# theadamsabra/last_torch

Hardware: AMD Instinct MI355X
Metric: lattice cells/s (B·T·U·|ctx|) at T=1000,U=100; 1/2/4/8-GPU scaling (higher is better)
Workload: dtype f32; 1 GPU; Log-semiring forward-backward (loss + dW), B=64/GPU, T=1000, U=100, V=32, FullNGram n=1 (C=33), fp32 (BASELINE configs[1]; configs[2] at 8 GPUs); batch_per_gpu=64, global_batch=64, frames=1000, labels=100, vocab=32, context_size=1, context_states=33, parallelism=utterance-sharded x1 (LPT), one RCCL all-reduce per step

## Files before the change

last_torch_amd/csrc/lt_chunk.hip:

```cpp
#include "lt_kernels.h"

#include <unistd.h>

#include <atomic>
#include <chrono>

namespace {

typedef float v16f __attribute__((ext_vector_type(16)));

constexpr float kEmin = 0x1p-88f;
constexpr int kRec = 1248;
constexpr int kRowT = 36;
constexpr int kChunkLds = 40 * 1024;
constexpr int kMargWaves = 4;
constexpr int kGrp = 7;
constexpr float kCert = 64.f;
#ifndef LT_AB_WAVES
#define LT_AB_WAVES 3
#endif
constexpr int kAbWaves = LT_AB_WAVES;
#ifndef LT_CK_APF
#define LT_CK_APF 1
#endif
constexpr int kApf = LT_CK_APF;
static_assert(kApf == 1 || kApf == 2, "phase A prefetch depth");
constexpr unsigned kSpinMax = 1u << 20;
#ifndef LT_CK_SPLIT
#define LT_CK_SPLIT 0
#endif
#ifndef LT_CK_WPRIO
#define LT_CK_WPRIO 3
#endif
#ifndef LT_CK_PRIO
#define LT_CK_PRIO 3
#endif
#ifndef LT_CK_ROT
#define LT_CK_ROT 1
#endif
#ifndef LT_CK_PF
#define LT_CK_PF 0
#endif
#ifndef LT_CK_NOACQ
#define LT_CK_NOACQ 1
#endif
constexpr bool kNoAcq = LT_CK_NOACQ != 0;
#ifndef LT_CK_ALDS
#define LT_CK_ALDS 1
#endif
constexpr bool kALds = LT_CK_ALDS != 0;
constexpr int kASlot = 5 * 1024;
constexpr int kALdsBytes = 4 * 2 * kASlot;
#ifndef LT_CK_BANDMIX
#define LT_CK_BANDMIX 0
#endif
constexpr bool kBandMix = LT_CK_BANDMIX != 0;
#ifndef LT_CK_EPIPE
#define LT_CK_EPIPE 0
#endif
constexpr bool kEpipe = LT_CK_EPIPE != 0;
#ifndef LT_WALK_SLOTS
#define LT_WALK_SLOTS 3
#endif
constexpr int kWalkSlots = LT_WALK_SLOTS;
constexpr int kRecNi = (4 * kRec + 1023) / 1024;
constexpr int kWalkSlot = kRecNi * 1024;
constexpr int kWalkLds = 2 * kWalkSlots * kWalkSlot;
constexpr int kRecEj = 1152, kRecRt = 1184, kRecRho = 1216, kRecPi = 1217, kRecCs = 1218,
              kRecFlag = 1219, kRecN = 1220;

struct CkArgs {
  const unsigned char* W;
  const int* nfr;
  const int* labels;
  const int* nlab;
  const float* grad;
  float* rec;
  float* nb;
  int* uflag;
  float* abd;
  float* bbd;
  float* nabd;
  float* nbbd;
  float* cf;
  unsigned long long* ready;
  unsigned long long* prog;
  unsigned long long ep_tag, pg_tag;
  float* mid;
  float* loss;
  float* log_z;
  float* num;
  float* lz_out;
  float* num_out;
  void* dW;
  int B, T, U, V, C, R, FR, NP, NPG, PPL, CP;
  int L, K;
  int NGc;
  int nc, wpos;
  int nbs;
  int half;
  int cont;
  int local;
  int strict;
  int dbg;
  int pf;
  long long* stamps;
  long long FB;
  int a_slots, a_ni, a_slot_bytes, a_wave_bytes, a_off_rt, a_off_tab;
  int b_ni, b_slots, b_off_ra, b_off_rb, b_off_ga, b_off_gb, b_gslots, b_gslot, b_off_buf;
  int c_ni, c_off_ad, c_off_bd, c_off_an, c_off_bn, c_off_nw, c_off_fs, c_off_tab, c_off_cf,
      c_off_buf, c_off_fl, c_off_e, c_bytes;
};

LT_DEVINL float half_sum(float v) {
  auto p = __builtin_amdgcn_permlane32_swap(__float_as_int(v), __float_as_int(v), false, false);
  return __int_as_float(p[0]) + __int_as_float(p[1]);
}
LT_DEVINL float half_other(float v) {
  auto p = __builtin_amdgcn_permlane32_swap(__float_as_int(v), __float_as_int(v), false, false);
  return (threadIdx.x & 32) ? __int_as_float(p[0]) : __int_as_float(p[1]);
}
LT_DEVINL float from_prev(float v, float fill) {
  return __int_as_float(
      __builtin_amdgcn_update_dpp(__float_as_int(fill), __float_as_int(v), 0x138, 0xF, 0xF, false));
}
LT_DEVINL float rot_prev(float v) {
  return __int_as_float(__builtin_amdgcn_update_dpp(0, __float_as_int(v), 0x13C, 0xF, 0xF, false));
}
LT_DEVINL float rot_next(float v) {
  return __int_as_float(__builtin_amdgcn_update_dpp(0, __float_as_int(v), 0x134, 0xF, 0xF, false));
}

LT_DEVINL float safe_max(float m) { return __builtin_isfinite(m) ? m : 0.f; }
#ifdef LT_DIAG
#define CK_STAMP(k)                                                                  \
  do {                                                                               \
    if (a.stamps && !LT_ABL(a, 64 | 256) && threadIdx.x == 0)                         \
      a.stamps[(long long)blockIdx.x * 8 + (k)] = (long long)__builtin_amdgcn_s_memtime(); \
  } while (0)
#define CK_WSTAMP(k)                                                                 \
  do {                                                                               \
    if (a.stamps && LT_ABL(a, 64) && (threadIdx.x & 63) == 0)                         \
      a.stamps[(long long)b * 8 + (k)] = (long long)__builtin_amdgcn_s_memtime();     \
  } while (0)
#define CK_ASTAMP(k)                                                                 \
  do {                                                                               \
    if (a.stamps && LT_ABL(a, 256) && (threadIdx.x & 63) == 0)                        \
      a.stamps[(long long)a.B * a.K * 8 + (long long)id * 4 + (k)] =                  \
          (long long)__builtin_amdgcn_s_memtime();                                   \
  } while (0)
#else
#define CK_ASTAMP(k) \
  do {               \
  } while (0)
#define CK_WSTAMP(k) \
  do {               \
  } while (0)
#define CK_STAMP(k) \
  do {              \
  } while (0)
#endif
LT_DEVINL float max3_raw(float x, float y, float z) {
  float r;
  asm("v_max3_f32 %0, %1, %2, %3" : "=v"(r) : "v"(x), "v"(y), "v"(z));
  return r;
}
LT_DEVINL float first_lane(float v) {
  return __int_as_float(__builtin_amdgcn_readfirstlane(__float_as_int(v)));
}

LT_DEVINL int kstep(int s, int h) { return (s & 3) + 8 * (s >> 2) + 4 * h; }

template <bool BF16>
LT_DEVINL float ldsw(const unsigned char* fr, int e) {
  if constexpr (BF16) return __uint_as_float(((unsigned)((const unsigned short*)fr)[e]) << 16);
  else return ((const float*)fr)[e];
}

LT_DEVINL void dma_issue(const unsigned char* base, long long off, long long bytes,
                         unsigned lds_addr, int ni, int lane, int wave0 = 0, int nwaves = 1,
                         bool sc1 = false) {
  const long long a0 = off & ~15LL;
  const int n16 = (int)((off + bytes - a0 + 15) >> 4);
  for (int i = wave0; i < ni; i += nwaves) {
    int g = lane + 64 * i;
    g = g < n16 ? g : n16 - 1;
    if (sc1) glds16_sc1(base + a0 + 16LL * g, lds_addr + 1024u * i);
    else glds16(base + a0 + 16LL * g, lds_addr + 1024u * i);
  }
}

LT_DEVINL void pf_lines(const unsigned char* base, long long off, long long bytes,
                        unsigned lds_addr, int lane) {
  const long long a0 = off & ~127LL;
  const int nl = (int)((off + bytes - a0 + 127) >> 7);
  lds_addr = __builtin_amdgcn_readfirstlane(lds_addr);
  for (int i = 0; 64 * i < nl; ++i) {
    const int g = min(lane + 64 * i, nl - 1);
    const void* src = base + a0 + 128LL * g;
    unsigned keep;
    asm volatile(
        "s_mov_b32 %0, m0\n\t"
        "s_mov_b32 m0, %2\n\t"
        "s_nop 0\n\t"
        "global_load_lds_dword %1, off\n\t"
        "s_mov_b32 m0, %0"
        : "=&s"(keep)
        : "v"(src), "s"(lds_addr)
        : "memory");
  }
}

LT_DEVINL void dma_range(const unsigned char* base, long long off, long long bytes,
// ... 873 lines not shown
      if (lane == 0) a.mid[2LL * b] = O;
    } else {
      if (wt) prog_publish(a, b, 0, k1 - Kh, lane);
      const float x = lane < C ? al : -kInf;
      const float M = safe_max(wmax_u(x));
      const float s = wsum_u(lane < C ? __builtin_amdgcn_exp2f(x - M) : 0.f);
      if (lane == 0)
        *wl.lz = (float)(((double)O + (double)(M + __builtin_amdgcn_logf(s))) * 0.6931471805599453);
    }
  } else if (wave == 1 && !a.local && !LT_ABL(a, 1)) {
    float* bc = wl.bc + 64;
    const int h = lane >> 5;
    float* dst = a.bbd + (long long)b * (a.K + 1) * CP;
    const int k0 = ph == kWalkFirst ? Kh : 0, k1 = ph == kWalkRest ? Kh : Kl;
    float be;
    if (ph == kWalkRest) {
      const float x = dst[(long long)Kh * CP + min(lane, C - 1)];
      be = lane < C ? x : -kInf;
    } else {
      be = lane < C ? 0.f : -kInf;
      if (lane < C) dst[(long long)Kl * CP + lane] = be;
    }
    int pub = 0;
    if (k1 > k0) {
      rd.ensure_bwd(k1 - kWalkSlots, lane);
      for (int n = 0; n < kWalkSlots; ++n) issue_rec(k1 - 1 - n, n);
    }
    for (int n = 0; n < k1 - k0; ++n) {
      const int k = k1 - 1 - n;
      wait_rec(n);
      RecBeta R;
      load_rec_beta(slot(n), lane, R);
      const float xc = (lane >= 1 && lane < C) ? be : -kInf;
      const float Mc = safe_max(wmax_u(xc));
      if (lane >= 1 && lane <= 32) bc[lane - 1] = lane < C ? __builtin_amdgcn_exp2f(xc - Mc) : 0.f;
      __builtin_amdgcn_s_waitcnt(0xc07f);
      __builtin_amdgcn_wave_barrier();
      float p0 = 0.f, p1 = 0.f;
#pragma unroll
      for (int g = 0; g < 4; ++g) {
        const float4 b4 = *(const float4*)(bc + 8 * g + 4 * h);
        p0 = __builtin_fmaf(R.x[4 * g + 0], b4.x, p0);
        p1 = __builtin_fmaf(R.x[4 * g + 1], b4.y, p1);
        p0 = __builtin_fmaf(R.x[4 * g + 2], b4.z, p0);
        p1 = __builtin_fmaf(R.x[4 * g + 3], b4.w, p1);
      }
      const float rp = lane < 32 ? R.rt * bc[lane & 31] : 0.f;
      const float ej = R.ej, rho = R.rho, pi = R.pi;
      __builtin_amdgcn_s_waitcnt(0xc07f);
      rd.ensure_bwd(k - kWalkSlots, lane);
      issue_rec(k - kWalkSlots, n + kWalkSlots);
      const float fl = floorf(Mc);
      const float tot = half_sum(p0 + p1);
      const float nj = (Mc - fl) + ej + __builtin_amdgcn_logf(tot);
      const float rsum = wsum_u(rp);
      const float rterm = (Mc - fl) + rho + __builtin_amdgcn_logf(rsum);
      const float nb0 = lse2_b2(first_lane(be) + pi - fl, rterm);
      const float sh = from_prev(nj, -kInf);
      be = lane == 0 ? nb0 : (lane < C ? sh : -kInf);
      if (lane < C) bd_store(dst + (long long)k * CP + lane, be, wt);
      if (wt && Kh - k - pub >= kProgStep && k > k0) {
        prog_publish(a, b, 1, Kh - k, lane);
        pub = Kh - k;
      }
      __builtin_amdgcn_wave_barrier();
    }
    if (wt) prog_publish(a, b, 1, Kh - k0, lane);
  } else if (wave == 2 && !LT_ABL(a, 2) && !LT_ABL(a, 128)) {
    num_walk<PPL, true, D>(a, b, lane, nf, Kl, nl, wl.nva, wl.num, rd, ph);
  } else if (wave == 3 && !LT_ABL(a, 2)) {
    num_walk<PPL, false, D>(a, b, lane, nf, Kl, nl, wl.nvb, nullptr, rd, ph);
  }
  if (lane == 0 && (rd.bad || !rd.ok)) *wl.bad = 1;
  CK_WSTAMP(2 * wave + 1);
  __syncthreads();
  if (ph == kWalkFirst) {
    if (threadIdx.x == 0) a.uflag[b] = *wl.bad ? 1 : 0;
    return;
  }
  if (*wl.bad) {
    if (threadIdx.x == 0) a.uflag[b] = 1;
    return;
  }
  if (threadIdx.x == 0) {
    const float lz = a.local ? 0.f : *wl.lz;
    const float nm = *wl.num;
    if (ph == kWalkRest && ((!a.local && !__builtin_isfinite(lz)) || !__builtin_isfinite(nm)))
      a.uflag[b] = 1;
    else if (ph == kWalkFull)
      a.uflag[b] = 0;
    a.log_z[b] = lz;
    a.num[b] = nm;
    if (a.lz_out) a.lz_out[b] = lz;
    if (a.num_out) a.num_out[b] = nm;
    a.loss[b] = a.local ? -nm : lz - nm;
  }
}

template <int PPL>
constexpr int kWalkD = PPL == 1 ? 8 : (kAbWaves > 3 ? 4 : 5);
template <int PPL>
constexpr int kWalkDc = PPL == 1 ? 4 : 3;

template <bool BF16, int PPL, bool FULL>
__global__ __launch_bounds__(256, kAbWaves) void ck_ab_kernel(const CkArgs a) {
  const int nc = a.nc;
  const int wave = __builtin_amdgcn_readfirstlane(threadIdx.x >> 6);
  int x = blockIdx.x;
  if (x >= a.wpos && x < a.wpos + nc) {
    extern __shared__ __attribute__((aligned(16))) unsigned char ck_dyn[];
    if (LT_CK_WPRIO) __builtin_amdgcn_s_setprio(LT_CK_WPRIO);
    combine_role<PPL, kWalkD<PPL>>(a, x - a.wpos, wave, ck_dyn, a.half ? kWalkFirst : kWalkFull);
    return;
  }
  if (x >= a.wpos) x -= nc;
  const long long j = (long long)x * 4 + wave;
  const int m = (int)(j / (2 * a.B));
  const int r = (int)(j - (long long)m * 2 * a.B);
  const int b = r < a.B ? r : r - a.B;
  int nf = a.nfr[b];
  nf = nf < 0 ? 0 : (nf > a.T ? a.T : nf);
  const int Kl = (nf + a.L - 1) / a.L;
  const int k = r < a.B ? m : Kl - 1 - m;
  if (r < a.B ? m > Kl - 1 - m : Kl - 1 - m <= m) return;
  transfer_role<BF16, PPL, FULL>(a, b, k, wave);
}

template <int PPL>
__global__ __launch_bounds__(256) void ck_combine_kernel(const CkArgs a) {
  extern __shared__ __attribute__((aligned(16))) unsigned char ck_dyn[];
  combine_role<PPL, kWalkD<PPL>>(a, blockIdx.x, __builtin_amdgcn_readfirstlane(threadIdx.x >> 6),
                                 ck_dyn, a.half ? kWalkFirst : kWalkFull);
}

LT_DEVINL void gather_tables(const CkArgs& a, int b, int* lab, int* boff, int* loff, int tid,
                             int nthr) {
  for (int j = tid; j < a.U; j += nthr) lab[j] = a.labels[(long long)b * a.U + j];
  __syncthreads();
  for (int u = tid; u < a.NPG; u += nthr) {
    int bo, lo;
    string_offsets(a, lab, u, &bo, &lo);
    boff[u] = bo < 0 ? 0 : bo;
    loff[u] = lo;
  }
}

template <bool BF16>
LT_DEVINL void store_dw(void* dW, long long e, float v) {
  if constexpr (BF16) ((unsigned short*)dW)[e] = f2bf(v);
  else ((float*)dW)[e] = v;
}

constexpr int kFs = 8, kFsMa = 0, kFsA0 = 1, kFsMb = 2, kFsB0 = 3, kFsW00 = 4;
constexpr int kFlA = 1, kFlB = 2, kFlNA = 4, kFlNB = 8, kFlAll = 15;

template <bool BF16, int PPL, bool FULL>
__global__ __launch_bounds__(64 * kMargWaves, kMargWaves / 2) void ck_marg_kernel(const CkArgs a) {
  extern __shared__ __attribute__((aligned(16))) unsigned char lds[];
  const int tid = threadIdx.x, lane = tid & 63;
  const int wave = __builtin_amdgcn_readfirstlane(tid >> 6);
  if (a.cont && (int)blockIdx.x < a.B) {
    CK_STAMP(0);
    if (LT_CK_WPRIO) __builtin_amdgcn_s_setprio(LT_CK_WPRIO);
    combine_role<PPL, kWalkDc<PPL>>(a, blockIdx.x, wave, lds, kWalkRest);
    CK_STAMP(4);
    return;
  }
  const int c = a.cont ? (int)blockIdx.x - a.B : (int)blockIdx.x;
  const int j = c / a.B, b = c - j * a.B;
  if (a.uflag[b]) return;
  int nf = a.nfr[b];
  nf = nf < 0 ? 0 : (nf > a.T ? a.T : nf);
  const int Kl = (nf + a.L - 1) / a.L, Kh = Kl / 2;
  const int k = j < 2 * Kh ? ((j & 1) ? Kh - 1 - (j >> 1) : Kh + (j >> 1)) : j;
  const int t0 = k * a.L;
  const int tend = min(t0 + a.L, a.T);
  const int t1 = max(t0, min(t0 + a.L, nf));
  const int V = FULL ? 32 : a.V, C = V + 1, R = V + 1, FR = C * R, CP = FULL ? 36 : a.CP;
  const int NPG = a.NPG, NP = a.NP;
  const int FRP = (FR + 3) & ~3;
  float g = a.grad ? a.grad[b] : 1.f;
  if (!a.cont) {
    const float lz = a.log_z[b], nm = a.num[b];
    if ((!a.local && !__builtin_isfinite(lz)) || __builtin_isnan(nm)) {
      if (tid == 0) a.uflag[b] = 1;
      return;
    }
    if (!__builtin_isfinite(nm)) g = 0.f;
  }
  const long long e0 = ((long long)b * a.T + t0) * FR;
  if (t1 <= t0 || g == 0.f) {
    const long long n = (long long)(tend - t0) * FR;
    for (long long e = tid; e < n; e += blockDim.x) store_dw<BF16>(a.dW, e0 + e, 0.f);
    return;
  }
  const int nt = t1 - t0;
  CK_STAMP(0);
  const int role = LT_CK_ROT == 1 ? (wave + (int)(blockIdx.x >> 3)) & 3
                 : LT_CK_ROT == 2 ? (wave + (int)blockIdx.x) & 3 : wave;
  const bool split = LT_CK_SPLIT && !a.local && !LT_ABL(a, 4 | 8);
  const int hs = (nt + 1) / 2;
  const long long off = e0 * (BF16 ? 2 : 4);
  if (!split) {
    dma_issue(a.W, off, (long long)nt * a.FB, lds_base_addr(lds), a.c_ni, lane, wave, kMargWaves);
  } else if (role < 2) {
    const int n1 = (int)(((off & 15) + (long long)hs * a.FB + 1023) >> 10);
    dma_range(a.W, off, (long long)nt * a.FB, lds_base_addr(lds), role == 0 ? 0 : max(n1 - 1, 0),
              role == 0 ? n1 : a.c_ni, lane);
  }
  unsigned char* wch = lds + (off & 15);
  float* xa = (float*)(lds + a.c_off_ad);
  float* xb = (float*)(lds + a.c_off_bd);
  float* an = (float*)(lds + a.c_off_an);
  float* bn = (float*)(lds + a.c_off_bn);
  float2* nw = (float2*)(lds + a.c_off_nw);
  float* fs = (float*)(lds + a.c_off_fs);
  int* boff = (int*)(lds + a.c_off_tab);
  int* loff = boff + NPG;
  int* labs = loff + NPG;
  float* buf = (float*)(lds + a.c_off_buf) + 64 * wave;
  float* cfl = (float*)(lds + a.c_off_cf);
  int* fl = (int*)(lds + a.c_off_fl);
  int* ford = fl + a.L;
  int* njob = ford + a.L;
  int* cert_fail = njob + 1;
  auto init_flags = [&](int t) {
    if (t < nt) {
      fl[t] = 0;
      const int mid = (nt - 1) / 2;
      const int k = (t + 1) / 2;
      ford[t] = (t & 1) ? mid + k : mid - k;
    }
    if (t == 0) {
      *njob = 0;
      *cert_fail = 0;
    }
  };
  if (split && role >= 2) {
    const int t2 = (role - 2) * 64 + lane;
    if (t2 < nt) cfl[t2] = a.cf[(long long)b * a.T + t0 + t2];
    for (int j = lane; j < a.U; j += 64) labs[j] = a.labels[(long long)b * a.U + j];
    __builtin_amdgcn_s_waitcnt(0xc07f);
    for (int u = t2; u < NPG; u += 128) {
      int bo, lo;
      string_offsets(a, labs, u, &bo, &lo);
      boff[u] = bo < 0 ? 0 : bo;
      loff[u] = lo;
    }
    init_flags(t2);
  }
  if (!split && tid < nt) cfl[tid] = a.cf[(long long)b * a.T + t0 + tid];
  if (a.cont && (split ? (role == 2 && lane == 0) : tid == 0)) {
    const int need_a = k - Kh, need_b = Kh - (k + 1);
    const unsigned long long* pg = a.prog + 4LL * b;
    int ok = 1;
    for (unsigned spins = 0;; ++spins) {
      bool done = true;
      if (need_a > 0)
        done = (a.local || prog_count(poll_flag(pg + 0), a.pg_tag) >= need_a) &&
               prog_count(poll_flag(pg + 2), a.pg_tag) >= need_a;
      if (done && need_b > 0)
        done = (a.local || prog_count(poll_flag(pg + 1), a.pg_tag) >= need_b) &&
               prog_count(poll_flag(pg + 3), a.pg_tag) >= need_b;
      if (done) break;
      if (spins > kSpinMax) {
        ok = 0;
        break;
      }
      __builtin_amdgcn_s_sleep(2);
    }
    if (!kNoAcq) acquire_agent();
    CK_STAMP(6);
    fl[2 * a.L + 2] = ok;
  }
  if (!split) {
    gather_tables(a, b, labs, boff, loff, tid, blockDim.x);
    wait_vmcnt(0);
    __syncthreads();
  } else {
    __builtin_amdgcn_s_waitcnt(0xc07f);
    __builtin_amdgcn_s_barrier();
    __builtin_amdgcn_fence(__ATOMIC_ACQUIRE, "workgroup");
  }
  if (a.cont && !fl[2 * a.L + 2]) {
    if (tid == 0) a.uflag[b] = 1;
    return;
  }
  CK_STAMP(1);
  auto wrow = [&](int f) -> const unsigned char* { return wch + f * a.FB; };
  auto eptr = [&](int f) -> float* {
    return BF16 ? (float*)(lds + a.c_off_e) + f * FRP : (float*)(wch + f * a.FB);
  };
  auto ew = [](float w, float cl) -> float {
    return __builtin_amdgcn_exp2f(__builtin_fmaf(w, kLog2e, -cl));
  };
  if (!split) {
    float2 g2[4];
    const int nnw = nt * NPG;
#pragma unroll
    for (int i = 0; i < 4; ++i) {
      const int x = min(tid + 64 * kMargWaves * i, nnw - 1);
      const int f = x / NPG, u = x - f * NPG;
      const unsigned char* fr = wch + f * a.FB;
      const int lo = loff[u];
      const float wb = ldsw<BF16>(fr, boff[u]), wl = ldsw<BF16>(fr, max(lo, 0));
      g2[i] = make_float2(u < NP ? wb * kLog2e : -kInf, (u >= 1 && u < NP) ? wl * kLog2e : -kInf);
    }
    for (int x = tid + 4 * 64 * kMargWaves; x < nnw; x += 64 * kMargWaves) {
      const int f = x / NPG, u = x - f * NPG;
      const unsigned char* fr = wch + f * a.FB;
      const int lo = loff[u];
      const float wb = ldsw<BF16>(fr, boff[u]), wl = ldsw<BF16>(fr, max(lo, 0));
      nw[x] = make_float2(u < NP ? wb * kLog2e : -kInf, (u >= 1 && u < NP) ? wl * kLog2e : -kInf);
    }
#pragma unroll
    for (int i = 0; i < 4; ++i)
      if (tid + 64 * kMargWaves * i < nnw) nw[tid + 64 * kMargWaves * i] = g2[i];
  }
  if (!split) {
    if (tid < nt) fs[tid * kFs + kFsW00] = ldsw<BF16>(wch + tid * a.FB, 0) * kLog2e;
    init_flags(tid);
    __syncthreads();
  }
  auto own_arcs = [&](int f, const unsigned char* fr) -> float {
    for (int u = lane; u < NPG; u += 64) {
      const int lo = loff[u];
      const float wb = ldsw<BF16>(fr, boff[u]), wl = ldsw<BF16>(fr, max(lo, 0));
      nw[f * NPG + u] =
          make_float2(u < NP ? wb * kLog2e : -kInf, (u >= 1 && u < NP) ? wl * kLog2e : -kInf);
    }
    const float w = ldsw<BF16>(fr, 0) * kLog2e;
    if (lane == 0) fs[f * kFs + kFsW00] = w;
    return w;
  };
  CK_STAMP(5);

  auto mark = [&](int f, int bit) {
    __builtin_amdgcn_fence(__ATOMIC_RELEASE, "workgroup");
    if (lane == 0) __hip_atomic_fetch_or(fl + f, bit, __ATOMIC_RELAXED, __HIP_MEMORY_SCOPE_WORKGROUP);
  };
  auto mark_all = [&](int bit) {
    for (int f = 0; f < nt; ++f) mark(f, bit);
  };
  auto wait_bits = [&](int f, int want) {
    for (;;) {
      const int bits = __builtin_amdgcn_readfirstlane(
          __hip_atomic_load(fl + f, __ATOMIC_RELAXED, __HIP_MEMORY_SCOPE_WORKGROUP));
      if ((bits & want) == want) break;
      __builtin_amdgcn_s_sleep(1);
    }
    __builtin_amdgcn_fence(__ATOMIC_ACQUIRE, "workgroup");
  };

  if (LT_CK_PRIO && role < 2) __builtin_amdgcn_s_setprio(LT_CK_PRIO);
  if (role == 0 && !a.local && !LT_ABL(a, 4)) {
    const int q = lane & 31, h = lane >> 5;
    const int qe = min(q, V - 1) + 1;
    const bool core = lane >= 1 && lane <= V;
    const float* xp = a.abd + ((long long)b * (a.K + 1) + k) * CP + min(lane, C - 1);
    const float xr = kNoAcq ? ld_sc1(xp) : *xp;
    const float x0 = lane < C ? xr : -kInf;
    float a0 = first_lane(x0);
    float S = wmax_u(core ? x0 : -kInf);
    float al = (core && S != -kInf) ? __builtin_amdgcn_exp2f(x0 - S) : 0.f;
    if (split) wait_vmcnt(0);
    auto get_e = [&](int f, float* e, float& e32, float& eb, float& w00) {
      const unsigned char* fr = wrow(f);
      float* ef = eptr(f);
      const float cl = cfl[f];
      w00 = fs[f * kFs + kFsW00];
      if (f < hs) {
        if (split) w00 = own_arcs(f, fr);
#pragma unroll
        for (int m = 0; m < 16; ++m) e[m] = ldsw<BF16>(fr, min(16 * h + m, C - 1) * R + qe);
        e32 = ldsw<BF16>(fr, min(32, C - 1) * R + qe);
        eb = ldsw<BF16>(fr, qe * R);
#pragma unroll
        for (int m = 0; m < 16; ++m) e[m] = ew(e[m], cl);
        e32 = ew(e32, cl);
        eb = ew(eb, cl);
#pragma unroll
        for (int m = 0; m < 16; ++m) ef[min(16 * h + m, C - 1) * R + qe] = e[m];
        ef[min(32, C - 1) * R + qe] = e32;
        ef[qe * R] = eb;
        if (lane == 0) ef[0] = 0.f;
      } else {
        wait_bits(f, kFlB);
        if (split) w00 = fs[f * kFs + kFsW00];
#pragma unroll
        for (int m = 0; m < 16; ++m) e[m] = ef[min(16 * h + m, C - 1) * R + qe];
        e32 = ef[min(32, C - 1) * R + qe];
        eb = ef[qe * R];
      }
    };
    float e[16], e32 = 0.f, eb = 0.f, w00 = 0.f;
    if (kEpipe && nt > 0) get_e(0, e, e32, eb, w00);
    for (int f = 0; f < nt; ++f) {
      const float cl = cfl[f];
      if (!kEpipe || f >= hs) get_e(f, e, e32, eb, w00);
      const float mc = wmax_u(core ? al : 0.f);
      int ex;
      (void)frexpf(mc, &ex);
      const float Ma = safe_max(mc > 0.f ? fmaxf(a0, S + (float)ex) : a0);
      const float xv = lane == 0 ? __builtin_amdgcn_exp2f(a0 - Ma) : al * __builtin_amdgcn_exp2f(S - Ma);
      if (lane < 36) buf[lane] = xv;
      if (lane < C) xa[f * CP + lane] = xv;
      if (lane == 0) {
        fs[f * kFs + kFsMa] = Ma;
        fs[f * kFs + kFsA0] = a0;
      }
      float en[16], en32 = 0.f, enb = 0.f, wn00 = 0.f;
      if (kEpipe && f + 1 < hs) get_e(f + 1, en, en32, enb, wn00);
      __builtin_amdgcn_s_waitcnt(0xc07f);
      __builtin_amdgcn_wave_barrier();
      float s0 = 0.f, s1 = 0.f;
#pragma unroll
      for (int g4 = 0; g4 < 4; ++g4) {
        const float4 b4 = *(const float4*)(buf + 16 * h + 4 * g4);
        s0 = __builtin_fmaf(b4.x, e[4 * g4 + 0], s0);
        s1 = __builtin_fmaf(b4.y, e[4 * g4 + 1], s1);
        s0 = __builtin_fmaf(b4.z, e[4 * g4 + 2], s0);
        s1 = __builtin_fmaf(b4.w, e[4 * g4 + 3], s1);
      }
      s0 = __builtin_fmaf(h ? buf[32] : buf[qe], h ? e32 : eb, s0);
      const float sq = half_sum(s0 + s1);
      S = Ma + cl;
      a0 += w00;
      const float sh = from_prev(sq, 0.f);
      al = core ? sh : 0.f;
      __builtin_amdgcn_wave_barrier();
      mark(f, kFlA);
      if (kEpipe && f + 1 < hs) {
#pragma unroll
        for (int m = 0; m < 16; ++m) e[m] = en[m];
        e32 = en32;
        eb = enb;
        w00 = wn00;
      }
    }
  } else if (role == 1 && !a.local && !LT_ABL(a, 4)) {
    const int j = lane & 31, h = lane >> 5;
    const int pe = min(j, V - 1) + 1;
    const bool core = lane >= 1 && lane <= V;
    const float* xp = a.bbd + ((long long)b * (a.K + 1) + k + 1) * CP + min(lane, C - 1);
    const float xr = kNoAcq ? ld_sc1(xp) : *xp;
    const float x0 = lane < C ? xr : -kInf;
    float b0 = first_lane(x0);
    float S = safe_max(wmax_u(core ? x0 : -kInf));
    float be = core ? __builtin_amdgcn_exp2f(x0 - S) : 0.f;
    if (split) wait_vmcnt(0);
    auto get_e = [&](int f, float* e, float& eb, float& e0y, float& w00) {
      const unsigned char* fr = wrow(f);
      float* ef = eptr(f);
      const float cl = cfl[f];
      w00 = fs[f * kFs + kFsW00];
      if (f >= hs) {
        if (split) w00 = own_arcs(f, fr);
#pragma unroll
        for (int m = 0; m < 16; ++m) e[m] = ldsw<BF16>(fr, pe * R + min(16 * h + m + 1, V));
        eb = ldsw<BF16>(fr, pe * R);
        e0y = ldsw<BF16>(fr, min(j, V - 1) + 1);
#pragma unroll
        for (int m = 0; m < 16; ++m) e[m] = ew(e[m], cl);
        eb = ew(eb, cl);
        e0y = ew(e0y, cl);
#pragma unroll
        for (int m = 0; m < 16; ++m) ef[pe * R + min(16 * h + m + 1, V)] = e[m];
        ef[pe * R] = eb;
        ef[min(j, V - 1) + 1] = e0y;
        if (lane == 0) ef[0] = 0.f;
      } else {
        wait_bits(f, kFlA);
        if (split) w00 = fs[f * kFs + kFsW00];
#pragma unroll
        for (int m = 0; m < 16; ++m) e[m] = ef[pe * R + min(16 * h + m + 1, V)];
        eb = ef[pe * R];
        e0y = ef[min(j, V - 1) + 1];
      }
    };
    float e[16], eb = 0.f, e0y = 0.f, w00 = 0.f;
    if (kEpipe && nt - 1 >= hs) get_e(nt - 1, e, eb, e0y, w00);
    for (int f = nt - 1; f >= 0; --f) {
      const float cl = cfl[f];
      if (!kEpipe || f < hs) get_e(f, e, eb, e0y, w00);
      const float mc = wmax_u(be);
      int ex;
      (void)frexpf(mc, &ex);
      const float Mb = mc > 0.f ? S + (float)ex : S;
      const float xv = be * __builtin_amdgcn_exp2f(S - Mb);
      if (lane >= 1 && lane <= 32) buf[lane - 1] = xv;
      if (lane < C) xb[f * CP + lane] = xv;
      if (lane == 0) {
        fs[f * kFs + kFsMb] = Mb;
        fs[f * kFs + kFsB0] = b0;
      }
      float en[16], enb = 0.f, en0y = 0.f, wn00 = 0.f;
      if (kEpipe && f - 1 >= hs) get_e(f - 1, en, enb, en0y, wn00);
      __builtin_amdgcn_s_waitcnt(0xc07f);
      __builtin_amdgcn_wave_barrier();
      float s0 = 0.f, s1 = 0.f;
#pragma unroll
      for (int g4 = 0; g4 < 4; ++g4) {
        const float4 b4 = *(const float4*)(buf + 16 * h + 4 * g4);
        s0 = __builtin_fmaf(b4.x, e[4 * g4 + 0], s0);
        s1 = __builtin_fmaf(b4.y, e[4 * g4 + 1], s1);
        s0 = __builtin_fmaf(b4.z, e[4 * g4 + 2], s0);
        s1 = __builtin_fmaf(b4.w, e[4 * g4 + 3], s1);
      }
      const float bj = buf[j];
      s0 = __builtin_fmaf(h ? 0.f : bj, eb, s0);
      const float sj = half_sum(s0 + s1);
      const float r0 = wsum_u(lane < 32 ? bj * e0y : 0.f);
      b0 = lse2_b2(b0 + w00, Mb + cl + __builtin_amdgcn_logf(r0));
      S = Mb + cl;
      const float sh = from_prev(sj, 0.f);
      be = core ? sh : 0.f;
      __builtin_amdgcn_wave_barrier();
      mark(f, kFlB);
      if (kEpipe && f - 1 >= hs) {
#pragma unroll
        for (int m = 0; m < 16; ++m) e[m] = en[m];
        eb = enb;
        e0y = en0y;
        w00 = wn00;
      }
    }
  } else if (role == 2 && !LT_ABL(a, 8)) {
    float al[PPL];
    const float* src = a.nabd + ((long long)b * (a.K + 1) + k) * NPG;
#pragma unroll
    for (int r = 0; r < PPL; ++r) {
      const int u = lane + 64 * r, uc = min(u, NPG - 1);
      const float v = kNoAcq ? ld_sc1(src + uc) : src[uc];
      al[r] = u < NPG ? v : -kInf;
    }
    for (int f = 0; f < nt; ++f) {
      if (split) wait_bits(f, f < hs ? kFlA : kFlB);
      float prev = -kInf, nv[PPL];
#pragma unroll
      for (int r = 0; r < PPL; ++r) {
        const int u = lane + 64 * r;
        if (u < NPG) an[f * NPG + u] = al[r];
        const float x = rot_prev(al[r]);
        const float pv = lane == 0 ? prev : x;
        prev = x;
        const float2 w = nw[f * NPG + min(u, NPG - 1)];
        nv[r] = lse2_b2(al[r] + w.x, pv + w.y);
      }
#pragma unroll
      for (int r = 0; r < PPL; ++r) al[r] = nv[r];
      __builtin_amdgcn_wave_barrier();
      mark(f, kFlNA);
    }
  } else if (role == 3 && !LT_ABL(a, 8)) {
    float be[PPL];
    const float* src = a.nbbd + ((long long)b * (a.K + 1) + k + 1) * NPG;
#pragma unroll
    for (int r = 0; r < PPL; ++r) {
      const int u = lane + 64 * r, uc = min(u, NPG - 1);
      const float v = kNoAcq ? ld_sc1(src + uc) : src[uc];
      be[r] = u < NPG ? v : -kInf;
    }
    if (a.pf) {
      const int c2 = c + a.pf;
      if (c2 < a.B * a.K) {
        const int j2 = c2 / a.B, b2 = c2 - j2 * a.B;
        int nf2 = a.nfr[b2];
        nf2 = nf2 < 0 ? 0 : (nf2 > a.T ? a.T : nf2);
        const int Kl2 = (nf2 + a.L - 1) / a.L, Kh2 = Kl2 / 2;
        const int k2 = j2 < 2 * Kh2 ? ((j2 & 1) ? Kh2 - 1 - (j2 >> 1) : Kh2 + (j2 >> 1)) : j2;
        const int t02 = k2 * a.L, t12 = max(t02, min(t02 + a.L, nf2));
        if (t12 > t02)
          pf_lines(a.W, ((long long)b2 * a.T + t02) * FR * (BF16 ? 2 : 4),
                   (long long)(t12 - t02) * a.FB, lds_base_addr((unsigned char*)buf), lane);
      }
    }
    for (int f = nt - 1; f >= 0; --f) {
      if (split) wait_bits(f, f < hs ? kFlA : kFlB);
      float nx[PPL], nv[PPL];
#pragma unroll
      for (int r = 0; r < PPL; ++r) nx[r] = rot_next(be[r]);
#pragma unroll
      for (int r = 0; r < PPL; ++r) {
        const int u = lane + 64 * r;
        if (u < NPG) bn[f * NPG + u] = be[r];
        const float nb = lane == 63 ? (r + 1 < PPL ? nx[r + 1 < PPL ? r + 1 : r] : -kInf) : nx[r];
        const float wb = nw[f * NPG + min(u, NPG - 1)].x;
        const float wl = nw[f * NPG + min(u + 1, NPG - 1)].y;
        nv[r] = lse2_b2(wb + be[r], (u + 1 < NP ? wl : -kInf) + nb);
      }
#pragma unroll
      for (int r = 0; r < PPL; ++r) be[r] = nv[r];
      __builtin_amdgcn_wave_barrier();
      mark(f, kFlNB);
    }
  } else {
    mark_all(role == 0 ? kFlA : role == 1 ? kFlB : role == 2 ? kFlNA : kFlNB);
  }
  if (LT_CK_PRIO && role < 2) __builtin_amdgcn_s_setprio(0);
  CK_STAMP(2);

  constexpr int NROW = 17;
  const int y = lane & 31, h = lane >> 5;
  const bool ycol = y < R;
  int bo[PPL], lo[PPL];
#pragma unroll
  for (int r = 0; r < PPL; ++r) {
    const int uc = min(lane + 64 * r, NP - 1);
    bo[r] = boff[uc];
    lo[r] = max(loff[uc], 0);
  }
  for (;;) {
    int jb = 0;
    if (lane == 0) jb = __hip_atomic_fetch_add(njob, 1, __ATOMIC_RELAXED, __HIP_MEMORY_SCOPE_WORKGROUP);
    jb = __builtin_amdgcn_readfirstlane(jb);
    if (jb >= nt || LT_ABL(a, 16)) break;
    const int f = ford[jb];
    for (;;) {
      const int bits = __builtin_amdgcn_readfirstlane(
          __hip_atomic_load(fl + f, __ATOMIC_RELAXED, __HIP_MEMORY_SCOPE_WORKGROUP));
      if ((bits & kFlAll) == kFlAll) break;
      __builtin_amdgcn_s_sleep(1);
    }
    __builtin_amdgcn_fence(__ATOMIC_ACQUIRE, "workgroup");
    float* fb = eptr(f);
    float sb[PPL], sl[PPL];
    float mxn = -kInf;
#pragma unroll
    for (int r = 0; r < PPL; ++r) {
      const int u = lane + 64 * r, uc = min(u, NP - 1);
      const float bu = bn[f * NPG + uc];
      const float2 w = nw[f * NPG + uc];
      const float tb = an[f * NPG + uc] + w.x + bu;
      const float tl = an[f * NPG + max(uc - 1, 0)] + w.y + bu;
      sb[r] = u < NP ? tb : -kInf;
      sl[r] = (u >= 1 && u < NP) ? tl : -kInf;
      mxn = fmaxf(mxn, fmaxf(sb[r], sl[r]));
    }
    mxn = safe_max(wmax_u(mxn));
    float zn = 0.f;
#pragma unroll
    for (int r = 0; r < PPL; ++r) {
      sb[r] = __builtin_amdgcn_exp2f(sb[r] - mxn);
      sl[r] = __builtin_amdgcn_exp2f(sl[r] - mxn);
      zn += sb[r] + sl[r];
    }
    zn = wsum_u(zn);
    const float gn = zn > 0.f ? g / zn : 0.f;
    if (!a.local) {
      const float* xaf = xa + f * CP;
      const float* xbf = xb + f * CP;
      const int yc = min(y, R - 1);
      const float xby = xbf[yc];
      float t[NROW], ra[NROW], rb[NROW];
#pragma unroll
      for (int m = 0; m < NROW; ++m) t[m] = fb[min(2 * m + h, C - 1) * R + yc];
#pragma unroll
      for (int m = 0; m < NROW; ++m) ra[m] = xaf[min(2 * m + h, C - 1)];
#pragma unroll
      for (int m = 0; m < NROW; ++m) rb[m] = xbf[min(2 * m + h, C - 1)];
      const int pc = min(lane, C - 1);
      float tc = fb[pc * R + (R - 1)] * xaf[pc] * xbf[R - 1];
      const bool colc = R == 33 && lane < 33;
      tc = colc ? tc : 0.f;
      float sum = tc;
#pragma unroll
      for (int m = 0; m < NROW; ++m) {
        const bool live = ycol && 2 * m + h < C && (R < 33 || y < 32);
        const float v = t[m] * ra[m] * (y ? xby : rb[m]);
        t[m] = live ? v : 0.f;
        sum += t[m];
      }
      sum = wsum_u(sum);
      const float* fsf = fs + f * kFs;
      const float base = fsf[kFsMa] + fsf[kFsMb] + cfl[f];
      const float v00 = fsf[kFsA0] + fsf[kFsW00] + fsf[kFsB0];
      const float zl = lse2_b2(base + __builtin_amdgcn_logf(sum), v00);
      if (!(base - zl <= kCert) && lane == 0) *cert_fail = 1;
      const float mult = g * __builtin_amdgcn_exp2f(base - zl);
      const float m00 = g * __builtin_amdgcn_exp2f(v00 - zl);
      __builtin_amdgcn_s_waitcnt(0xc07f);
      __builtin_amdgcn_wave_barrier();
#pragma unroll
      for (int m = 0; m < NROW; ++m) {
        const int p = 2 * m + h;
        if (ycol && p < C && (R < 33 || y < 32))
          fb[p * R + y] = (m == 0 && lane == 0) ? m00 : t[m] * mult;
      }
      if (colc) fb[pc * R + (R - 1)] = tc * mult;
    } else {
      __builtin_amdgcn_s_waitcnt(0xc07f);
      __builtin_amdgcn_wave_barrier();
      for (int e = lane; e < FR; e += 64) fb[e] = 0.f;
    }
#pragma unroll
    for (int r = 0; r < PPL; ++r) {
      const int u = lane + 64 * r;
      if (u < NP) {
        atomicAdd(fb + bo[r], -sb[r] * gn);
        if (u >= 1) atomicAdd(fb + lo[r], -sl[r] * gn);
      }
    }
    __builtin_amdgcn_s_waitcnt(0xc07f);
    __builtin_amdgcn_wave_barrier();
    if constexpr (BF16) {
      unsigned short* fo = (unsigned short*)(wch + f * a.FB);
      for (int e = lane; e < FR; e += 64) fo[e] = f2bf(fb[e]);
    }
  }
  __syncthreads();
  if (*cert_fail) {
    if (tid == 0) a.uflag[b] = 1;
    return;
  }
  CK_STAMP(3);
  {
    const long long es = BF16 ? 2 : 4;
    const long long bytes = (long long)nt * a.FB;
    unsigned char* gdst = (unsigned char*)a.dW + off;
    const long long head = min((long long)((16 - (off & 15)) & 15), bytes);
    const long long body = (bytes - head) & ~15LL;
    const unsigned char* src = wch;
    for (long long x = tid; x < head / es; x += blockDim.x) {
      if constexpr (BF16) ((unsigned short*)gdst)[x] = ((const unsigned short*)src)[x];
      else ((float*)gdst)[x] = ((const float*)src)[x];
    }
    const uint4* s16 = (const uint4*)(src + head);
    uint4* d16 = (uint4*)(gdst + head);
    for (long long x = tid; x < body / 16; x += blockDim.x) d16[x] = s16[x];
    for (long long x = head + body + tid * es; x < bytes; x += blockDim.x * es) {
      if constexpr (BF16) *(unsigned short*)(gdst + x) = *(const unsigned short*)(src + x);
      else *(float*)(gdst + x) = *(const float*)(src + x);
    }
  }
  CK_STAMP(4);
  {
    const long long n = (long long)(tend - t1) * FR;
    const long long base = e0 + (long long)nt * FR;
    for (long long e = tid; e < n; e += blockDim.x) store_dw<BF16>(a.dW, base + e, 0.f);
  }
}

}

namespace {

int ck_env(const char* name, int dflt) { return lt_impl::tune_int(name, dflt); }
long long up256(long long x) { return (x + 255) & ~255LL; }
int al16(long long x) { return (int)((x + 15) & ~15LL); }

struct CkLayout {
  size_t uflag, lz, num, abd, bbd, nabd, nbbd, cf, mid, state;
  size_t ready, rec, nb, f_alpha, f_an, f_loss, f_lz, f_num, f_side, scratch;
};

int ck_plan(const lt_problem* pb, int local_norm, CkArgs* a, CkLayout* w) {
  memset(a, 0, sizeof(*a));
  const int V = pb->vocab_size;
  const bool bf16 = pb->weight_dtype == LT_DTYPE_BF16;
  const int es = bf16 ? 2 : 4;
  a->B = pb->batch; a->T = pb->max_frames; a->U = pb->max_labels;
  a->V = V; a->C = V + 1; a->R = V + 1; a->FR = a->C * a->R;
  a->NP = a->U + 1; a->NPG = (a->NP + 1) & ~1; a->PPL = (a->NPG + 63) / 64;
  a->CP = (a->C + 3) & ~3;
  a->local = local_norm ? 1 : 0;
#ifdef LT_DIAG
  a->dbg = ck_env("LT_CK_DBG", 0);
  a->pf = ck_env("LT_CK_PF", LT_CK_PF);
  if (const char* sp = lt_impl::tune_str("LT_CK_STAMPS")) a->stamps = (long long*)strtoull(sp, nullptr, 0);
#endif
  a->FB = (long long)a->FR * es;
  const long long n16f = (a->FB + 30) / 16;
  a->a_ni = (int)((n16f + 63) / 64);
  a->a_slots = 3;
  a->a_slot_bytes = a->a_ni * 1024;
  a->a_off_rt = a->a_slots * a->a_slot_bytes;
  a->a_off_tab = a->a_off_rt + 128;
  a->a_wave_bytes = al16(a->a_off_tab + 8LL * a->NPG);
  a->b_ni = (kRec * 4 + 15 + 1023) / 1024;
  a->b_slots = 4;
  a->b_off_ra = 0;
  a->b_off_rb = a->b_slots * a->b_ni * 1024;
  a->b_gslot = 1024;
  a->b_gslots = 16;
  a->b_off_ga = a->b_off_rb + a->b_slots * a->b_ni * 1024;
  a->b_off_gb = a->b_off_ga + a->b_gslots * a->b_gslot;
  a->b_off_buf = a->b_off_gb + a->b_gslots * a->b_gslot;
  auto c_bytes = [&](int L, CkArgs* t) {
    const long long n16 = ((long long)L * a->FB + 30) / 16;
    t->c_ni = (int)((n16 + 63) / 64);
    int off = t->c_ni * 1024;
    t->c_off_ad = off; off += al16(4LL * L * a->CP);
    t->c_off_bd = off; off += al16(4LL * L * a->CP);
    t->c_off_an = off; off += al16(4LL * L * a->NPG);
    t->c_off_bn = off; off += al16(4LL * L * a->NPG);
    t->c_off_nw = off; off += al16(8LL * L * a->NPG);
    t->c_off_fs = off; off += al16(4LL * L * kFs);
    t->c_off_tab = off; off += al16(8LL * a->NPG + 4LL * a->U);
    t->c_off_cf = off; off += al16(4LL * L);
    t->c_off_buf = off; off += 4 * 64 * 4;
    t->c_off_fl = off; off += al16(4LL * (2 * L + 3));
    t->c_off_e = off; off += bf16 ? al16(4LL * L * ((a->FR + 3) & ~3)) : 0;
    return off;
  };
  int L = std::max(1, std::min(32, ck_env("LT_CHUNK_LEN", 32)));
  const int budget = ck_env("LT_CHUNK_LDS", kChunkLds);
  while (L > 4 && c_bytes(L, a) > budget) --L;
  if (c_bytes(L, a) > 160 * 1024) return lt_impl::set_error(LT_EUNSUPPORTED, "chunk: LDS");
  a->c_bytes = c_bytes(L, a);
  a->L = L;
  a->K = std::max(1, (a->T + L - 1) / L);
  if (a->K >= (1 << 24)) return lt_impl::set_error(LT_EUNSUPPORTED, "chunk: too many frames");
  a->NGc = (L + kGrp - 1) / kGrp;
  const long long B = a->B, K = a->K, T = a->T;
  size_t o = 0;
  w->uflag = o; o += up256(4 * B);
  w->lz = o; o += up256(4 * B);
  w->num = o; o += up256(4 * B);
  w->abd = o; o += up256(4 * B * (K + 1) * a->CP);
  w->bbd = o; o += up256(4 * B * (K + 1) * a->CP);
  w->nabd = o; o += up256(4 * B * (K + 1) * a->NPG);
  w->nbbd = o; o += up256(4 * B * (K + 1) * a->NPG);
  w->cf = o; o += up256(4 * B * T);
  w->mid = o; o += up256(8 * B);
  w->state = o;
  size_t s = 0;
  w->ready = s; s += up256(8LL * B * K + 32LL * B);
  w->rec = s; s += up256(4LL * B * K * kRec);
  a->nbs = (a->NGc * (kGrp + 1) * a->NPG + 31) & ~31;
  w->nb = s; s += up256(4LL * B * K * a->nbs);
  const size_t fwd = s;
  s = 0;
  w->f_alpha = s; s += up256(4LL * B * T * a->C);
  w->f_an = s; s += up256(4LL * B * T * a->NP);
  w->f_loss = s; s += up256(4 * B);
  w->f_lz = s; s += up256(4 * B);
  w->f_num = s; s += up256(4 * B);
  w->f_side = s; s += up256((long long)lt_impl::serial_side_bytes(pb, local_norm));
  w->scratch = std::max(fwd, s);
  return LT_OK;
}

void ck_bind(CkArgs* a, const CkLayout& w, void* state, void* scratch) {
  char* st = (char*)state;
  char* sc = (char*)scratch;
  a->uflag = (int*)(st + w.uflag);
  a->log_z = (float*)(st + w.lz);
  a->num = (float*)(st + w.num);
  a->abd = (float*)(st + w.abd);
  a->bbd = (float*)(st + w.bbd);
  a->nabd = (float*)(st + w.nabd);
  a->nbbd = (float*)(st + w.nbbd);
  a->cf = (float*)(st + w.cf);
// ... 243 lines not shown
```

Measured before the change: 660.1 billion cells/s.

## Precompute numerator terms for tail frames and restructure gradient gather layout

Beta-walk waves (role >= 2) now compute the numerator gradient terms for the last couple of frames ahead of time, store them in the an/bn buffers and set a new flag, so the marginal loop skips that work on the critical tail. The weight gather is reorganised so each thread handles a fixed label position across frames, which makes the boff/loff lookups loop-invariant. The denominator column computation is reorganised so each half-wave covers contiguous rows, allowing float4 loads of xa and dropping the rb array. These changes add new flag synchronisation and reuse of the an/bn buffers, and both carry correctness risk.

After: 681.2 billion cells/s, median of 6. 1.03x the previous value.

```diff
diff --git a/last_torch_amd/csrc/lt_chunk.hip b/last_torch_amd/csrc/lt_chunk.hip
--- a/last_torch_amd/csrc/lt_chunk.hip
+++ b/last_torch_amd/csrc/lt_chunk.hip
@@ -59,6 +59,18 @@
 #define LT_CK_EPIPE 0
 #endif
 constexpr bool kEpipe = LT_CK_EPIPE != 0;
+#ifndef LT_CK_NTERM
+#define LT_CK_NTERM 2
+#endif
+constexpr int kNTerm = LT_CK_NTERM;
+#ifndef LT_CK_DENCOL
+#define LT_CK_DENCOL 2
+#endif
+constexpr int kDenCol = LT_CK_DENCOL;
+#ifndef LT_CK_GSHIFT
+#define LT_CK_GSHIFT 1
+#endif
+constexpr bool kGShift = LT_CK_GSHIFT != 0;
 #ifndef LT_WALK_SLOTS
 #define LT_WALK_SLOTS 3
 #endif
@@ -1238,7 +1250,7 @@
 }
 
 constexpr int kFs = 8, kFsMa = 0, kFsA0 = 1, kFsMb = 2, kFsB0 = 3, kFsW00 = 4;
-constexpr int kFlA = 1, kFlB = 2, kFlNA = 4, kFlNB = 8, kFlAll = 15;
+constexpr int kFlA = 1, kFlB = 2, kFlNA = 4, kFlNB = 8, kFlAll = 15, kFlNT = 16;
 
 template <bool BF16, int PPL, bool FULL>
 __global__ __launch_bounds__(64 * kMargWaves, kMargWaves / 2) void ck_marg_kernel(const CkArgs a) {
@@ -1380,7 +1392,31 @@
   auto ew = [](float w, float cl) -> float {
     return __builtin_amdgcn_exp2f(__builtin_fmaf(w, kLog2e, -cl));
   };
-  if (!split) {
+  if (!split && kGShift) {
+    constexpr int PW = 64 * PPL, FPP = 64 * kMargWaves / PW, NU = PPL == 1 ? 2 : 3;
+    const int u = tid & (PW - 1), f0 = tid / PW;
+    const int uc = min(u, NPG - 1);
+    const int ob = boff[uc], ol = max(loff[uc], 0);
+    const bool inb = u < NP, inl = u >= 1 && u < NP;
+    const int FBi = (int)a.FB;
+    float2 g2[NU];
+#pragma unroll
+    for (int i = 0; i < NU; ++i) {
+      const unsigned char* fr = wch + min(FPP * i + f0, nt - 1) * FBi;
+      const float wb = ldsw<BF16>(fr, ob), wl = ldsw<BF16>(fr, ol);
+      g2[i] = make_float2(inb ? wb * kLog2e : -kInf, inl ? wl * kLog2e : -kInf);
+    }
+    for (int f = FPP * NU + f0; f < nt; f += FPP) {
+      const unsigned char* fr = wch + f * FBi;
+      const float wb = ldsw<BF16>(fr, ob), wl = ldsw<BF16>(fr, ol);
+      if (u < NPG) nw[f * NPG + u] = make_float2(inb ? wb * kLog2e : -kInf, inl ? wl * kLog2e : -kInf);
+    }
+#pragma unroll
+    for (int i = 0; i < NU; ++i) {
+      const int f = FPP * i + f0;
+      if (f < nt && u < NPG) nw[f * NPG + u] = g2[i];
+    }
+  } else if (!split) {
     float2 g2[4];
     const int nnw = nt * NPG;
 #pragma unroll
@@ -1686,31 +1722,7 @@
   if (LT_CK_PRIO && role < 2) __builtin_amdgcn_s_setprio(0);
   CK_STAMP(2);
 
-  constexpr int NROW = 17;
-  const int y = lane & 31, h = lane >> 5;
-  const bool ycol = y < R;
-  int bo[PPL], lo[PPL];
-#pragma unroll
-  for (int r = 0; r < PPL; ++r) {
-    const int uc = min(lane + 64 * r, NP - 1);
-    bo[r] = boff[uc];
-    lo[r] = max(loff[uc], 0);
-  }
-  for (;;) {
-    int jb = 0;
-    if (lane == 0) jb = __hip_atomic_fetch_add(njob, 1, __ATOMIC_RELAXED, __HIP_MEMORY_SCOPE_WORKGROUP);
-    jb = __builtin_amdgcn_readfirstlane(jb);
-    if (jb >= nt || LT_ABL(a, 16)) break;
-    const int f = ford[jb];
-    for (;;) {
-      const int bits = __builtin_amdgcn_readfirstlane(
-          __hip_atomic_load(fl + f, __ATOMIC_RELAXED, __HIP_MEMORY_SCOPE_WORKGROUP));
-      if ((bits & kFlAll) == kFlAll) break;
-      __builtin_amdgcn_s_sleep(1);
-    }
-    __builtin_amdgcn_fence(__ATOMIC_ACQUIRE, "workgroup");
-    float* fb = eptr(f);
-    float sb[PPL], sl[PPL];
+  auto num_terms = [&](int f, float* sb, float* sl) -> float {
     float mxn = -kInf;
 #pragma unroll
     for (int r = 0; r < PPL; ++r) {
@@ -1732,30 +1744,131 @@
       zn += sb[r] + sl[r];
     }
     zn = wsum_u(zn);
-    const float gn = zn > 0.f ? g / zn : 0.f;
+    return zn > 0.f ? g / zn : 0.f;
+  };
+  const int jpre = kNTerm == 1 ? 0 : max(nt - 2, 0);
+  if (kNTerm && role >= 2) {
+    for (int jb = jpre + role - 2; jb < nt; jb += 2) {
+      const int f = ford[jb];
+      wait_bits(f, kFlNA | kFlNB);
+      float sb[PPL], sl[PPL];
+      const float gn = num_terms(f, sb, sl);
+      __builtin_amdgcn_s_waitcnt(0xc07f);
+      __builtin_amdgcn_wave_barrier();
+#pragma unroll
+      for (int r = 0; r < PPL; ++r) {
+        const int u = lane + 64 * r;
+        if (u < NP) {
+          an[f * NPG + u] = -sb[r] * gn;
+          bn[f * NPG + u] = -sl[r] * gn;
+        }
+      }
+      __builtin_amdgcn_wave_barrier();
+      mark(f, kFlNT);
+    }
+  }
+
+  constexpr int NROW = 17;
+  const int y = lane & 31, h = lane >> 5;
+  const bool ycol = y < R;
+  int bo[PPL], lo[PPL];
+#pragma unroll
+  for (int r = 0; r < PPL; ++r) {
+    const int uc = min(lane + 64 * r, NP - 1);
+    bo[r] = boff[uc];
+    lo[r] = max(loff[uc], 0);
+  }
+  for (;;) {
+    int jb = 0;
+    if (lane == 0) jb = __hip_atomic_fetch_add(njob, 1, __ATOMIC_RELAXED, __HIP_MEMORY_SCOPE_WORKGROUP);
+    jb = __builtin_amdgcn_readfirstlane(jb);
+    if (jb >= nt || LT_ABL(a, 16)) break;
+    const int f = ford[jb];
+    const bool pre = kNTerm && jb >= jpre;
+    const int want = pre ? (kFlA | kFlB | kFlNT) : kFlAll;
+    for (;;) {
+      const int bits = __builtin_amdgcn_readfirstlane(
+          __hip_atomic_load(fl + f, __ATOMIC_RELAXED, __HIP_MEMORY_SCOPE_WORKGROUP));
+      if ((bits & want) == want) break;
+      __builtin_amdgcn_s_sleep(1);
+    }
+    __builtin_amdgcn_fence(__ATOMIC_ACQUIRE, "workgroup");
+    float* fb = eptr(f);
+    float sb[PPL], sl[PPL];
+    if (pre) {
+#pragma unroll
+      for (int r = 0; r < PPL; ++r) {
+        const int uc = min(lane + 64 * r, NP - 1);
+        sb[r] = an[f * NPG + uc];
+        sl[r] = bn[f * NPG + uc];
+      }
+    } else {
+      const float gn = num_terms(f, sb, sl);
+#pragma unroll
+      for (int r = 0; r < PPL; ++r) {
+        sb[r] = -sb[r] * gn;
+        sl[r] = -sl[r] * gn;
+      }
+    }
     if (!a.local) {
       const float* xaf = xa + f * CP;
       const float* xbf = xb + f * CP;
-      const int yc = min(y, R - 1);
-      const float xby = xbf[yc];
-      float t[NROW], ra[NROW], rb[NROW];
-#pragma unroll
-      for (int m = 0; m < NROW; ++m) t[m] = fb[min(2 * m + h, C - 1) * R + yc];
-#pragma unroll
-      for (int m = 0; m < NROW; ++m) ra[m] = xaf[min(2 * m + h, C - 1)];
-#pragma unroll
-      for (int m = 0; m < NROW; ++m) rb[m] = xbf[min(2 * m + h, C - 1)];
+      float t[NROW], ra[NROW], tc, sum;
+      bool colc;
       const int pc = min(lane, C - 1);
-      float tc = fb[pc * R + (R - 1)] * xaf[pc] * xbf[R - 1];
-      const bool colc = R == 33 && lane < 33;
-      tc = colc ? tc : 0.f;
-      float sum = tc;
-#pragma unroll
-      for (int m = 0; m < NROW; ++m) {
-        const bool live = ycol && 2 * m + h < C && (R < 33 || y < 32);
-        const float v = t[m] * ra[m] * (y ? xby : rb[m]);
-        t[m] = live ? v : 0.f;
-        sum += t[m];
+      if constexpr (kDenCol != 0) {
+        const int yq = min(y + 1, R - 1);
+        const bool yl = y + 1 < R;
+        const float xby = xbf[yq];
+        const float eb = fb[pc * R], xap = xaf[pc], xbp = xbf[pc];
+#pragma unroll
+        for (int m = 0; m < 16; ++m) t[m] = fb[min(16 * h + m, C - 1) * R + yq];
+        t[16] = fb[min(32, C - 1) * R + yq];
+        if constexpr (FULL && kDenCol == 2) {
+#pragma unroll
+          for (int g4 = 0; g4 < 4; ++g4) {
+            const float4 x4 = *(const float4*)(xaf + 16 * h + 4 * g4);
+            ra[4 * g4 + 0] = x4.x;
+            ra[4 * g4 + 1] = x4.y;
+            ra[4 * g4 + 2] = x4.z;
+            ra[4 * g4 + 3] = x4.w;
+          }
+        } else {
+#pragma unroll
+          for (int m = 0; m < 16; ++m) ra[m] = xaf[min(16 * h + m, C - 1)];
+        }
+        ra[16] = xaf[min(32, C - 1)];
+        colc = lane < C;
+        tc = colc ? eb * xap * xbp : 0.f;
+        sum = tc;
+#pragma unroll
+        for (int m = 0; m < NROW; ++m) {
+          const bool live = yl && (m < 16 ? 16 * h + m < C : (h == 1 && C > 32));
+          const float v = t[m] * ra[m] * xby;
+          t[m] = live ? v : 0.f;
+          sum += t[m];
+        }
+      } else {
+        const int yc = min(y, R - 1);
+        const float xby = xbf[yc];
+        float rb[NROW];
+#pragma unroll
+        for (int m = 0; m < NROW; ++m) t[m] = fb[min(2 * m + h, C - 1) * R + yc];
+#pragma unroll
+        for (int m = 0; m < NROW; ++m) ra[m] = xaf[min(2 * m + h, C - 1)];
+#pragma unroll
+        for (int m = 0; m < NROW; ++m) rb[m] = xbf[min(2 * m + h, C - 1)];
+        tc = fb[pc * R + (R - 1)] * xaf[pc] * xbf[R - 1];
+        colc = R == 33 && lane < 33;
+        tc = colc ? tc : 0.f;
+        sum = tc;
+#pragma unroll
+        for (int m = 0; m < NROW; ++m) {
+          const bool live = ycol && 2 * m + h < C && (R < 33 || y < 32);
+          const float v = t[m] * ra[m] * (y ? xby : rb[m]);
+          t[m] = live ? v : 0.f;
+          sum += t[m];
+        }
       }
       sum = wsum_u(sum);
       const float* fsf = fs + f * kFs;
@@ -1767,13 +1880,22 @@
       const float m00 = g * __builtin_amdgcn_exp2f(v00 - zl);
       __builtin_amdgcn_s_waitcnt(0xc07f);
       __builtin_amdgcn_wave_barrier();
-#pragma unroll
-      for (int m = 0; m < NROW; ++m) {
-        const int p = 2 * m + h;
-        if (ycol && p < C && (R < 33 || y < 32))
-          fb[p * R + y] = (m == 0 && lane == 0) ? m00 : t[m] * mult;
-      }
-      if (colc) fb[pc * R + (R - 1)] = tc * mult;
+      if constexpr (kDenCol != 0) {
+#pragma unroll
+        for (int m = 0; m < NROW; ++m) {
+          const int p = m < 16 ? 16 * h + m : 32;
+          if (y + 1 < R && (m < 16 ? p < C : (h == 1 && C > 32))) fb[p * R + y + 1] = t[m] * mult;
+        }
+        if (colc) fb[pc * R] = lane == 0 ? m00 : tc * mult;
+      } else {
+#pragma unroll
+        for (int m = 0; m < NROW; ++m) {
+          const int p = 2 * m + h;
+          if (ycol && p < C && (R < 33 || y < 32))
+            fb[p * R + y] = (m == 0 && lane == 0) ? m00 : t[m] * mult;
+        }
+        if (colc) fb[pc * R + (R - 1)] = tc * mult;
+      }
     } else {
       __builtin_amdgcn_s_waitcnt(0xc07f);
       __builtin_amdgcn_wave_barrier();
@@ -1783,8 +1905,8 @@
     for (int r = 0; r < PPL; ++r) {
       const int u = lane + 64 * r;
       if (u < NP) {
-        atomicAdd(fb + bo[r], -sb[r] * gn);
-        if (u >= 1) atomicAdd(fb + lo[r], -sl[r] * gn);
+        atomicAdd(fb + bo[r], sb[r]);
+        if (u >= 1) atomicAdd(fb + lo[r], sl[r]);
       }
     }
     __builtin_amdgcn_s_waitcnt(0xc07f);
```
